# Seasandwpy/viso

Measured on AMD Instinct MI355X. Metric: stereo frames/sec at 1242x375 grey, 1/2/4/8 GPUs; pose RMSE vs reference, higher is better.
Workload: dtype f64

## Files before the change

viso_amd/csrc/context.hip:

```cpp
#include <algorithm>
#include <cstdio>
#include <cstring>
#include <new>
#include <vector>

#include "context.hpp"

using namespace viso;

namespace viso {

int DevBuf::ensure(size_t need) {
    if (need <= bytes) return VISO_OK;
    if (ptr) {
        VISO_HIP_CHECK(hipFree(ptr));
        ptr = nullptr;
        bytes = 0;
    }
    size_t b = std::max<size_t>(need, 256);
    VISO_HIP_CHECK(hipMalloc(&ptr, b));
    bytes = b;
    return VISO_OK;
}

// ... 60 lines not shown
int viso_create(const viso_params* p, int device, viso_ctx** out) {
    if (!p || !out) return VISO_ERR_ARG;
    *out = nullptr;
    if (p->width < 16 || p->height < 16 || p->width > kMaxWidth) return VISO_ERR_ARG;
    if (p->max_features <= 0 || p->max_features > 65536 || p->batch_frames <= 0) return VISO_ERR_ARG;
    if (p->precision != VISO_PRECISION_FAITHFUL && p->precision != VISO_PRECISION_FAST) return VISO_ERR_ARG;
    int rc = check_device_present();
    if (rc != VISO_OK) return rc;
    VISO_HIP_CHECK(hipSetDevice(device));
    viso_ctx* c = new (std::nothrow) viso_ctx();
    if (!c) return VISO_ERR_ARG;
    c->p = *p;
    c->device = device;
    if (const char* e = getenv("VISO_HOST_TIMES")) c->host_times.on = c->stage.timed = e[0] == '1';
    if (const char* e = getenv("VISO_HOST_TIMELINE")) c->dev_tl.on = e[0] == '1';
    c->geom = make_geom(p->width, p->height);
    if (c->create_streams() != VISO_OK) {
        delete c;
        return VISO_ERR_HIP;
    }
    rc = c->init();
    if (rc != VISO_OK) {
        viso_destroy(c);
        return rc;
    }
    *out = c;
    return VISO_OK;
}

int viso_destroy(viso_ctx* c) {
// ... 183 lines not shown
    if (rc) return rc;
    char* base = (char*)c->scratch_a.ptr;
    VISO_HIP_CHECK(hipMemcpyAsync(base + o_l, last_pyr, g.bytes, hipMemcpyHostToDevice, c->stream));
    VISO_HIP_CHECK(hipMemcpyAsync(base + o_c, cur_pyr, g.bytes, hipMemcpyHostToDevice, c->stream));
    if (n > 0)
        VISO_HIP_CHECK(hipMemcpyAsync(base + o_p, points, 24 * (size_t)n, hipMemcpyHostToDevice, c->stream));
    VISO_HIP_CHECK(hipMemcpyAsync(base + o_pl, pose_last, 96, hipMemcpyHostToDevice, c->stream));
    VISO_HIP_CHECK(hipMemcpyAsync(base + o_pio, pose_io, 96, hipMemcpyHostToDevice, c->stream));
    const double K[4] = {c->p.fx, c->p.fy, c->p.cx, c->p.cy};
    {
        TimedRegion t(c->timing, VISO_KERNEL_DIRECT, c->stream);
        launch_direct_pose(frame_from_base((const uint8_t*)(base + o_l), g),
                           frame_from_base((const uint8_t*)(base + o_c), g), g, K,
                           (const double*)(base + o_p), n, (const double*)(base + o_pl),
                           (const double*)(base + o_pio), direct_scratch_at(base + o_ds), nullptr,
                           (double*)(base + o_pio), nullptr, -1, c->stream, c->p.precision);
    }
    VISO_HIP_CHECK(hipGetLastError());
    VISO_HIP_CHECK(hipMemcpyAsync(pose_io, base + o_pio, 96, hipMemcpyDeviceToHost, c->stream));
    VISO_HIP_CHECK(hipStreamSynchronize(c->stream));
    return VISO_OK;
}

int viso_lk_align(viso_ctx* c, const uint8_t* kf_pyrs, const double* kf_poses, int32_t n_kf,
                  const uint8_t* cur_pyr, const double cur_pose[12], int32_t width, int32_t height,
                  const double* points, int32_t n, int32_t* pair_kf, uint8_t* success,
                  double* uv_before, double* uv_after) {
    if (!c || !kf_pyrs || !kf_poses || n_kf <= 0 || n_kf > kMaxKeyframes || !cur_pyr || !cur_pose ||
        n < 0)
        return VISO_ERR_ARG;
    if (int rc = c->settle()) return rc;
// ... 168 lines not shown
```

viso_amd/csrc/context.hpp:

```cpp
#pragma once

#include <chrono>
#include <deque>
#include <vector>

#include "../../include/viso/viso_c.h"
#include "geometry.hpp"
#include "kernels.hpp"
#include "staging.hpp"
#include "trace.hpp"

namespace viso {

struct DevBuf {
    void* ptr = nullptr;
    size_t bytes = 0;
    int ensure(size_t need);
    void release();
    template <class T>
    T* as() const { return (T*)ptr; }
};

struct Timing {
    bool enabled = false;
// ... 188 lines not shown
    viso::DevBuf map_pts;
    int n_map = 0;
    viso::DevBuf kf_poses;

    viso::DevBuf direct_buf;
    viso::DirectScratch direct{};
    viso::DevBuf direct_stats;
    std::vector<int> lk_pending;
    int lk_last_rows = 0;
    int lk_last_pts = 0;
    viso::DevBuf lk_pair, lk_succ, lk_before, lk_after;
    viso::DevBuf lk_tmpl, lk_tmpl_h, lk_tmpl_kf, lk_tmpl_uv;
    hipStream_t lk_stream = nullptr;
    hipEvent_t lk_ring[viso::kLkRing] = {};
    viso::HostStage stage;
    viso::HostTimes host_times;
    viso::DevTimeline dev_tl;
    hipStream_t up_stream = nullptr;
    int64_t epoch = 0;
    hipEvent_t epoch_evt[viso::kEpochRing] = {};
    int64_t epoch_rec_call[viso::kEpochRing] = {};
    int64_t epoch_nrec = 0;
    int64_t epoch_last_rec = -(1LL << 40);
    int wait_freed(int64_t fe, hipStream_t st);
    hipEvent_t epoch_now = nullptr;
    int end_epoch();
    int create_up_stream();
    int upload_host(int s, const uint8_t* grey, int32_t w, int32_t h, int32_t stride, bool pyramid);
    hipEvent_t geo_fork = nullptr, geo_join = nullptr;
    int64_t lk_seq = 0;
// ... 122 lines not shown
```

viso_amd/csrc/direct.hip:

```cpp
#include <algorithm>
#include <cstring>

#include "device_math.hpp"
#include "direct_solve.hpp"
#include "kernels.hpp"

#ifdef VISO_PROBE
constexpr int kPRing = 4096;
constexpr int kPSt = 16;
__device__ unsigned long long g_plog[kPRing][kPSt];
__device__ unsigned long long g_pexit[kPRing];
constexpr int kPRingB = 512;
__device__ unsigned long long g_pblk[kPRingB][256][4];
__device__ unsigned long long g_pwave[kPRingB][256][16];
#ifdef VISO_PROBE_PT
constexpr int kPtRing = 128, kPtBlocks = 32, kPtStamps = 5;
__device__ unsigned long long g_ppt[kPtRing][kPtBlocks][16][kPtStamps];
#define PPT(k)                                                                                       \
    do {                                                                                             \
        if (blockIdx.x < kPtBlocks && (threadIdx.x & 63) == 0)                                       \
            g_ppt[a.probe_seq & (kPtRing - 1)][blockIdx.x][threadIdx.x >> 6][(k)] =                  \
                __builtin_amdgcn_s_memrealtime();                                                    \
    } while (0)
#endif
// ... 266 lines not shown
            const int o = (iy - c.y0) * kCW + (ix - c.x0);
            const double d0 = (double)ld_lds_u8(win, o), d1 = (double)ld_lds_u8(win, o + 1);
            const double d2 = (double)ld_lds_u8(win, o + kCW), d3 = (double)ld_lds_u8(win, o + kCW + 1);
            const double xx = x - floor(x);
            const double yy = y - floor(y);
            return double((1 - xx) * (1 - yy) * d0 + xx * (1 - yy) * d1 + (1 - xx) * yy * d2 +
                          xx * yy * d3);
        }
    }
#ifdef VISO_PROBE
    PFB_ADD(w >= 1000 ? 0 : w >= 500 ? 1 : w >= 250 ? 2 : 3);
#endif
    return sample_px(img, w, h, x, y);
}

__device__ inline double point_quotients(const Intrinsics& K, const double* pose, const double* P, double scale,
                                         double* Q, double* qt) {
    const int lane = threadIdx.x & 63;
    double Pc[3];
    mat3_vec(pose, P, Pc);
    const double x = Pc[0] + pose[9], y = Pc[1] + pose[10], z = Pc[2] + pose[11];
    const double fx = K.fx * scale, fy = K.fy * scale;
    const double zz = z * z, xy = x * y;
    const double fxx = fx * x, fyy = fy * y;
    double c1, c2, den;
    if (qt) {
        if (lane == 0) {
            double2* t2 = reinterpret_cast<double2*>(qt);
            t2[0] = make_double2(x, y);
            t2[1] = make_double2(fx, -fx);
            t2[2] = make_double2(fxx, fy);
            t2[3] = make_double2(-fy, fyy);
            t2[4] = make_double2(1.0, xy);
            t2[5] = make_double2(z, zz);
        }
        __builtin_amdgcn_fence(__ATOMIC_RELEASE, "wavefront");
        __builtin_amdgcn_wave_barrier();
        __builtin_amdgcn_fence(__ATOMIC_ACQUIRE, "wavefront");
        constexpr unsigned long long kC1 = 0x557653433210ULL, kC2 = 0x091181090888ULL,
                                     kDen = 0xABBBAABBBAAAULL;
        const int l = lane < 12 ? lane : 11;
        c1 = qt[(kC1 >> (4 * l)) & 15];
        c2 = qt[(kC2 >> (4 * l)) & 15];
        den = qt[(kDen >> (4 * l)) & 15];
    } else {
        c1 = fy;
        c1 = lane == 0 ? x : c1;
        c1 = lane == 1 ? y : c1;
        c1 = lane == 2 ? fx : c1;
        c1 = (lane == 3 || lane == 4 || lane == 6) ? -fx : c1;
        c1 = lane == 5 ? fxx : c1;
        c1 = lane == 8 ? -fy : c1;
        c1 = lane == 9 ? fyy : c1;
        c2 = 1.0;
        c2 = (lane == 3 || lane == 5 || lane >= 11) ? x : c2;
        c2 = (lane == 4 || lane == 10) ? xy : c2;
        c2 = (lane == 6 || lane == 8 || lane == 9) ? y : c2;
        den = (lane <= 2 || lane == 6 || lane == 7 || lane >= 11) ? z : zz;
    }
    double q = (c1 * c2) / den;
    if (lane == 5) q = fx + q;
    if (lane == 9) q = -fy - q;
    Q[0] = readlane_f64(q, 0);
    Q[1] = readlane_f64(q, 1);
    return lane < 12 ? q : 0.0;
}

__device__ inline unsigned factored_sources() {
    const int k = threadIdx.x & 31;
    constexpr unsigned long long lo[4] = {0x43333ccccc222222ULL, 0x9888877777ccccccULL, 0x465436543c6543c2ULL,
                                          0x9ba98ba987ba987cULL};
    constexpr unsigned long long hi[4] = {0x26543c265544ULL, 0xcba987cbaa99ULL, 0xccccccc66565ULL,
                                          0x7777777bbabaULL};
    unsigned r = 0;
#pragma unroll
    for (int q = 0; q < 4; ++q)
        r |= (unsigned)((k < 16 ? lo[q] >> (4 * k) : hi[q] >> (4 * (k - 16))) & 15) << (8 * q);
// ... 11 lines not shown
        a[k] = ra + rb;
    }
    double ra, rb;
    permlane16_swap_f64(a[0], a[2], ra, rb);
    const double c0 = ra + rb;
    permlane16_swap_f64(a[1], a[1], ra, rb);
    const double c1 = ra + rb;
    double d = dsel(b3, c1, c0) + dpp_f64<0x128>(dsel(b3, c0, c1));
    const double r4 = dpp_f64<0x114>(d), l4 = dpp_f64<0x104>(d);
    d = d + dsel(b2, r4, l4);
    d = d + dpp_f64<0x4E>(d);
    d = d + dpp_f64<0xB1>(d);
    return d;
}

__device__ inline bool direct_point_rs(const DirectArgs& a, const LevelPair& fp, int lv,
                                       const double* cur_pose,
                                       const RefSample& r, const uint8_t* win, const CurWin& cw,
                                       double* out, int* idx, unsigned src_lanes, double* qt = nullptr) {
    const int lane = threadIdx.x & 63;
    const int px = (lane >> 3) - 4, py = (lane & 7) - 4;
    const double scale = kScale[lv];
    const int w = a.g.w[lv], h = a.g.h[lv];
    PPT(0);
    double Q[2];
    const double jq = point_quotients(a.K, cur_pose, r.P, scale, Q, qt);
    PPT(1);
    const double uc = scale * (Q[0] * a.K.fx + a.K.cx);
    const double vc = scale * (Q[1] * a.K.fy + a.K.cy);
    const double hp = 4.0;
    const bool good = r.ok && inside_px(uc - hp, vc - hp, w, h) && inside_px(uc + hp, vc + hp, w, h);
    if (!good) return false;
    const uint8_t* C = fp.cur;
    const double x = uc + px, y = vc + py;
    double error, g0, g1;
    const int fu = (int)floor(uc), fv = (int)floor(vc);
    if (__builtin_expect(cw.on && fu - 6 >= cw.x0 && fu + 5 <= cw.x0 + kCW - 2 && fv - 6 >= cw.y0 &&
                             fv + 5 <= cw.y0 + kCW - 2,
                         1)) {
        const bool one_binade = uc >= 6.0 && vc >= 6.0 &&
                                (__double_as_longlong(uc - 6.0) >> 52) == (__double_as_longlong(uc + 6.0) >> 52) &&
                                (__double_as_longlong(vc - 6.0) >> 52) == (__double_as_longlong(vc + 6.0) >> 52);
        if (__builtin_expect(one_binade, 1)) {
            const double xx = uc - floor(uc), yy = vc - floor(vc);
            const double w00 = (1 - xx) * (1 - yy), w10 = xx * (1 - yy), w01 = (1 - xx) * yy, w11 = xx * yy;
            const uint8_t* wb = win + ((fv + py - 1 - cw.y0) * kCW + (fu + px - 1 - cw.x0));
            auto tap = [&](int dx, int dy) { return (double)ld_lds_u8(wb, (dy + 1) * kCW + (dx + 1)); };
            const double tm0 = tap(-1, 0), t00 = tap(0, 0), t10 = tap(1, 0), t20 = tap(2, 0);
            const double tm1 = tap(-1, 1), t01 = tap(0, 1), t11 = tap(1, 1), t21 = tap(2, 1);
            const double t0m = tap(0, -1), t1m = tap(1, -1), t02 = tap(0, 2), t12 = tap(1, 2);
            auto bil = [&](double d0, double d1, double d2, double d3) {
                return double(w00 * d0 + w10 * d1 + w01 * d2 + w11 * d3);
            };
            error = r.lval - bil(t00, t10, t01, t11);
            g0 = 0.5 * (bil(t10, t20, t11, t21) - bil(tm0, t00, tm1, t01));
            g1 = 0.5 * (bil(t01, t11, t02, t12) - bil(t0m, t1m, t00, t10));
        } else {
            auto smp = [&](double sx, double sy) {
                const int o = ((int)sy - cw.y0) * kCW + ((int)sx - cw.x0);
                const double d0 = (double)ld_lds_u8(win, o), d1 = (double)ld_lds_u8(win, o + 1);
                const double d2 = (double)ld_lds_u8(win, o + kCW), d3 = (double)ld_lds_u8(win, o + kCW + 1);
                const double sxx = sx - floor(sx);
                const double syy = sy - floor(sy);
                return double((1 - sxx) * (1 - syy) * d0 + sxx * (1 - syy) * d1 + (1 - sxx) * syy * d2 +
                              sxx * syy * d3);
            };
            error = r.lval - smp(x, y);
            g0 = 0.5 * (smp(x + 1, y) - smp(x - 1, y));
            g1 = 0.5 * (smp(x, y + 1) - smp(x, y - 1));
        }
    } else {
        error = r.lval - sample_cw(C, w, h, x, y, win, cw);
        g0 = 0.5 * (sample_cw(C, w, h, x + 1, y, win, cw) - sample_cw(C, w, h, x - 1, y, win, cw));
        g1 = 0.5 * (sample_cw(C, w, h, x, y + 1, win, cw) - sample_cw(C, w, h, x, y - 1, win, cw));
    }
    PPT(2);
    const double leaf[6] = {g0 * g0, g0 * g1, g1 * g1, error * g0, error * g1, error * error};
    const double s = reduce_scatter_6_desc(leaf);
    PPT(3);
    const unsigned sa = src_lanes;
    const double p0a = bperm_f64(jq, (int)(sa & 0xff)), p1a = bperm_f64(jq, (int)((sa >> 8) & 0xff));
    const double p0b = bperm_f64(jq, (int)((sa >> 16) & 0xff)), p1b = bperm_f64(jq, (int)(sa >> 24));
    const double S0 = readlane_f64(s, 0), S1 = readlane_f64(s, 8), S2 = readlane_f64(s, 16);
    const double S3 = readlane_f64(s, 32), S4 = readlane_f64(s, 40), S5 = readlane_f64(s, 48);
    double o;
    if (lane < 21)
        o = (S0 * (p0a * p0b) + S1 * (p0a * p1b + p1a * p0b)) + S2 * (p1a * p1b);
    else if (lane < 27)
        o = S3 * p0a + S4 * p1a;
    else
        o = S5;
    *out = o;
    *idx = lane < kSums ? lane : -1;
    PPT(4);
    return true;
}

__device__ inline float tap_f32(const uint8_t* __restrict__ img, long long n, long long i) {
    return (float)ld_u8_or0(img, n, i);
}

__device__ inline bool direct_point_fast(const DirectArgs& a, const LevelPair& fp, int lv, const double* cur_pose,
                                         const double* P, float lval, const uint8_t* win, const CurWin& cw,
                                         float* out, int* idx) {
    const int lane = threadIdx.x & 63;
    const int px = (lane >> 3) - 4, py = (lane & 7) - 4;
    const double scale = kScale[lv];
    const int w = a.g.w[lv], h = a.g.h[lv];
    double Pc[3];
// ... 216 lines not shown
        const uint32_t t = pf.taps[j][lane];
        r.t0 = (int)(t & 0xff);
        r.t1 = (int)((t >> 8) & 0xff);
        r.t2 = (int)((t >> 16) & 0xff);
        r.t3 = (int)(t >> 24);
    } else {
        const uint8_t* img = fp.last;
        const long long n = (long long)w * (long long)h;
        r.t0 = ld_u8_or0(img, n, base);
        r.t1 = ld_u8_or0(img, n, base + 1);
        r.t2 = ld_u8_or0(img, n, base + w);
        r.t3 = ld_u8_or0(img, n, base + w + 1);
    }
}

constexpr unsigned kSrcHere = 0xffffffffu;

template <bool FAST, bool LV16 = false, int W = kWaves>
__device__ void direct_tile_pf(const DirectArgs& a, const LevelPair& fp, int lv, const double* cur_pose, int b,
                               const PfLds& pf, bool merged, double* part, int* good, double* s_pts,
                               int* s_good, int* s_cnt = nullptr, double* s_qt = nullptr,
                               unsigned src_in = kSrcHere) {
    const int wave = wave_id(), lane = threadIdx.x & 63;
    int first, T;
    tile_range(a, b, &first, &T);
    int good_cnt = 0;
    const unsigned src_lanes = FAST ? 0u : src_in != kSrcHere ? src_in : factored_sources();
    for (int local = wave; local < T; local += W) {
        const int i = first + local;
        double f = 0.0;
        int idx = -1;
        bool ok = false;
        if (i < a.n) {
            RefSample r;
            if (merged) {
                merged_ref(a, fp, lv, pf, local, r);
                if (!FAST) ref_finish(r);
            } else if (!FAST) {
                pf_ref(pf, local, r);
            } else {
                r.P[0] = pf.P[local][0];
                r.P[1] = pf.P[local][1];
// ... 8 lines not shown
                r.t3 = (int)(t >> 24);
            }
            CurWin cw;
            cw.x0 = pf.cw[local][0];
            cw.y0 = pf.cw[local][1];
            cw.on = pf.cw[local][2] != 0;
            if (FAST) {
                float ff = 0.0f;
                if (r.ok) {
                    const uint32_t t = (uint32_t)r.t0 | ((uint32_t)r.t1 << 8) | ((uint32_t)r.t2 << 16) |
                                       ((uint32_t)r.t3 << 24);
                    const float lval = (LV16 && !merged) ? (float)pf.lv16[local][lane] : fast_lval(t, r.ur, r.vr);
                    ok = direct_point_fast(a, fp, lv, cur_pose, r.P, lval, pf.win[local], cw, &ff, &idx);
                }
                f = (double)ff;
            } else {
                ok = direct_point_rs(a, fp, lv, cur_pose, r, pf.win[local], cw, &f, &idx, src_lanes,
                                     s_qt ? s_qt + 12 * wave : nullptr);
            }
        }
        if (!ok) {
            if (lane < kSums) s_pts[local * kSums + lane] = 0.0;
        } else if ((!FAST || lane < 32) && idx >= 0) {
            s_pts[local * kSums + idx] = f;
        }
        good_cnt += ok ? 1 : 0;
    }
    if (lane == 0 && good_cnt) atomicAdd(s_good, good_cnt);
#ifdef VISO_PROBE
    if (threadIdx.x == 0 && blockIdx.x < 256) g_pblk[a.probe_seq & (kPRingB - 1)][blockIdx.x][2] = __builtin_amdgcn_s_memrealtime();
// ... 137 lines not shown
            for (int k = 0; k < 7; ++k) a.s.state[kLevels * kStateStride + k] = L.state[k];
            if (a.prev_pose_out) store_frame_pose(a.prev_pose_out, s_last, a.prev_ready);
            log_pose(a.prev_log, a.prev_log_host, a.prev_log_index, s_last);
            log_frame(a.flog, a.prev_log_index, L);
        }
        double q[4];
        quat_from_matrix(s_last, q);
        for (int k = 0; k < 4; ++k) L.state[k] = q[k];
        L.state[4] = s_last[9];
        L.state[5] = s_last[10];
        L.state[6] = s_last[11];
    }
    state_to_pose(L.state, s_pose);
}

template <bool FAST>
__global__ __launch_bounds__(kThreads, 4) void direct_level_kernel(const double* __restrict__ pre_part,
                                                                 const int* __restrict__ pre_good, int pre_hdr,
                                                                 DirectArgs a) {
    PROBE_DECL();
    __builtin_amdgcn_s_setprio(1);
    __shared__ SolveLds L;
    __shared__ double s_pose[12];
    __shared__ double s_last[12];
    __shared__ double s_pts[kMaxTile * kSums];
    __shared__ int s_good;
    __shared__ int s_cnt;
    __shared__ int s_arrive;
    __shared__ PfLds s_pf;
#ifndef VISO_NO_QT
    __shared__ __attribute__((aligned(16))) double s_qt[FAST ? 2 : kWaves * 12];
    double* const qt = FAST ? nullptr : s_qt;
#else
    double* const qt = nullptr;
#endif
    const int lv = a.level;
    const bool merged = a.merged && lv == kLevels - 1;
    const int prev = lv + 1;
    const bool solve = prev < kLevels || merged;
    const int sl = merged ? 0 : prev;
    const int t = threadIdx.x, wave = t >> 6, lane = t & 63;
    const bool tiles = lv >= 0 && (int)blockIdx.x < a.n_tiles;
    double v[kSums];
    int gg = 0;
    if (((pre_hdr >> 16) & 1) && t < 256) load_partials(pre_part, pre_good, pre_hdr & 0xffff, v, gg);
    const bool pf_wave = !solve || (wave & 3) != 0;
    double st[7];
    if (t == 256 || (solve && tiles && pf_wave)) {
        if (!solve) {
            quat_from_matrix(a.pose_seed, st);
// ... 3 lines not shown
        } else {
#pragma unroll
            for (int k = 0; k < 7; ++k) st[k] = a.s.state[sl * kStateStride + k];
        }
    }
    if (t == 0) {
        s_arrive = 0;
        s_good = 0;
        s_cnt = 0;
#ifdef VISO_PROBE
        for (int k = 0; k < kPSt; ++k) pst[k] = 0;
        pst[0] = probe_t0;
        if (blockIdx.x < 256) g_pblk[a.probe_seq & (kPRingB - 1)][blockIdx.x][0] = probe_t0;
#endif
    }
    lds_barrier();

    if (t == 256) {
        for (int k = 0; k < 7; ++k) {
            L.state[k] = st[k];
            L.best[k] = st[k];
        }
        L.cost = 0.0;
        L.last_cost = 0.0;
        L.cont = 0;
        asm volatile("s_waitcnt lgkmcnt(0)" ::: "memory");
        atomicAdd(&s_arrive, 1);
    }
    if (solve && t < 256) {
        int idx;
// ... 82 lines not shown
        if (lv < 0 && a.pose_out) {
            store_frame_pose(a.pose_out, s_pose, a.ready);
            log_pose(a.log, a.log_host, a.log_index, s_pose);
            log_frame(a.flog, a.log_index, L);
        }
    }
    if (blockIdx.x == 0 && t == 0 && merged)
        for (int k = 0; k < 7; ++k) a.s.state[lv * kStateStride + k] = L.state[k];
    if (tiles) {
        LevelPair fp = level_pair(a.fp, lv);
        if (merged) fp.pose_last = s_last;
        double pose[12];
#pragma unroll
        for (int k = 0; k < 12; ++k) pose[k] = s_pose[k];
        direct_tile_pf<FAST>(a, fp, lv, pose, blockIdx.x, s_pf, merged, a.s.part + (size_t)lv * kMaxTiles * kSums,
                       a.s.good + lv * kMaxTiles, s_pts, &s_good, &s_cnt, qt, src_lanes);
    }
#ifdef VISO_PROBE
    __syncthreads();
    const unsigned long long t_exit = __builtin_amdgcn_s_memrealtime();
    const int slot = a.probe_seq & (kPRing - 1);
    if (t == 0 && blockIdx.x < 256) g_pblk[a.probe_seq & (kPRingB - 1)][blockIdx.x][3] = t_exit;
    if (blockIdx.x == 0 && t == 0) {
        pst[11] = t_exit;
        pst[15] = (unsigned long long)(lv + 1) | ((unsigned long long)merged << 8) |
                  ((unsigned long long)a.n_tiles << 16);
        for (int k = 0; k < kPSt; ++k) g_plog[slot][k] = pst[k];
    }
#endif
}

// ... 420 lines not shown
    }
    a.s = s;
    a.stats = stats;
    a.log_index = -1;
    a.prev_log_index = -1;
    return a;
}
}

bool direct_fits_background() { return kThreads <= 768; }

void launch_direct_levels(const FrameDev& last_pyr, const FrameDev& cur_pyr, const PyrGeom& g,
                          const double K[4], const double* points, int n,
                          const double* pose_last12, const double* pose_seed12,
                          const DirectScratch& s, double* stats, const DirectPrev* merge,
                          hipStream_t stream, int precision, bool bg) {
    DirectArgs a = direct_args(last_pyr, cur_pyr, g, K, points, n, pose_last12, pose_seed12, s,
                               stats, precision == VISO_PRECISION_FAST);
    if (merge) {
        a.merged = 1;
        a.prev.last = merge->last;
        a.prev.cur = merge->cur;
        a.prev.pose_last = merge->pose_last12;
        a.prev_pose_out = merge->pose_out;
        a.prev_log = merge->log;
        a.prev_log_index = merge->log ? merge->log_index : -1;
        a.prev_log_host = merge->log ? merge->log_host : nullptr;
        a.prev_ready = merge->ready;
        a.flog = merge->log ? merge->flog : nullptr;
    }
    const int grid = a.n_tiles > 0 ? a.n_tiles : 1;
    for (int level = kLevels - 1; level >= 0; --level) {
        a.level = level;
        a.probe_seq = next_probe_seq();
        const bool merged = a.merged && level == kLevels - 1;
        const bool solve = level + 1 < kLevels || merged;
        const int sl = merged ? 0 : level + 1;
        const double* pp = solve ? a.s.part + (size_t)sl * kMaxTiles * kSums : nullptr;
        const int* pg = solve ? a.s.good + sl * kMaxTiles : nullptr;
        const int hdr = a.n_tiles | (solve ? 1 << 16 : 0) | (bg ? kHdrBg : 0);
        if (precision == VISO_PRECISION_FAST)
            direct_level_kernel<true><<<grid, kThreads, 0, stream>>>(pp, pg, hdr, a);
        else
            direct_level_kernel<false><<<grid, kThreads, 0, stream>>>(pp, pg, hdr, a);
        a.merged = 0;
    }
}

void launch_direct_final(const FrameDev& last_pyr, const FrameDev& cur_pyr, const PyrGeom& g,
                         const double K[4], const double* points, int n,
                         const double* pose_last12, const DirectScratch& s, double* stats,
                         double* pose_out, double* log, int log_index, hipStream_t stream, int precision,
                         int* ready, double* log_host, double* flog) {
    DirectArgs a = direct_args(last_pyr, cur_pyr, g, K, points, n, pose_last12, pose_last12, s,
                               stats, precision == VISO_PRECISION_FAST);
    a.pose_out = pose_out;
    a.ready = ready;
// ... 103 lines not shown
            else
                rig_level_kernel<false, true><<<gl, kRigThreads, 0, stream>>>(psc, pad, hdr, t01, t23, ra);
        } else if (fast) {
            rig_level_kernel<true, false><<<gl, kRigThreads, 0, stream>>>(psc, pad, hdr, t01, t23, ra);
        } else {
            rig_level_kernel<false, false><<<gl, kRigThreads, 0, stream>>>(psc, pad, hdr, t01, t23, ra);
        }
    }
    return 0;
}

void launch_direct_pose(const FrameDev& last_pyr, const FrameDev& cur_pyr, const PyrGeom& g,
                        const double K[4], const double* points, int n,
                        const double* pose_last12, const double* pose_seed12,
                        const DirectScratch& s, double* stats, double* pose_out, double* log,
                        int log_index, hipStream_t stream, int precision) {
    launch_direct_levels(last_pyr, cur_pyr, g, K, points, n, pose_last12, pose_seed12, s, stats,
                         nullptr, stream, precision);
    launch_direct_final(last_pyr, cur_pyr, g, K, points, n, pose_last12, s, stats, pose_out, log,
                        log_index, stream, precision);
}

}

#ifdef VISO_PROBE
extern "C" int viso_debug_probe_ring(unsigned long long* log, unsigned long long* exits, int cap, int* n_launches,
                                     int reset) {
    using namespace viso;
    static unsigned long long hlog[kPRing][kPSt], hexit[kPRing];
    if (hipDeviceSynchronize() != hipSuccess) return -2;
    if (hipMemcpyFromSymbol(hlog, HIP_SYMBOL(g_plog), sizeof(hlog)) != hipSuccess) return -2;
    if (hipMemcpyFromSymbol(hexit, HIP_SYMBOL(g_pexit), sizeof(hexit)) != hipSuccess) return -2;
    const int n = (int)g_probe_host_seq;
// ... 86 lines not shown
```

viso_amd/csrc/frame.hip:

```cpp
#include <algorithm>
#include <cstdio>
#include <cstring>
#include <vector>

#include "context.hpp"

using namespace viso;

namespace {

void eigen_inverse3(const double* m, double* inv) {
    auto M = [&](int i, int j) { return m[3 * i + j]; };
    auto cof = [&](int i, int j) {
        int i1 = (i + 1) % 3, i2 = (i + 2) % 3, j1 = (j + 1) % 3, j2 = (j + 2) % 3;
        return M(i1, j1) * M(i2, j2) - M(i1, j2) * M(i2, j1);
    };
    double c0[3] = {cof(0, 0), cof(1, 0), cof(2, 0)};
    double det = (c0[0] * M(0, 0) + c0[1] * M(1, 0)) + c0[2] * M(2, 0);
    double invdet = 1.0 / det;
    inv[0] = c0[0] * invdet;
    inv[1] = c0[1] * invdet;
    inv[2] = c0[2] * invdet;
    inv[3] = cof(0, 1) * invdet;
    inv[4] = cof(1, 1) * invdet;
// ... 1082 lines not shown
                if (dpend) {
                    m.last = frame(dpend_last);
                    m.cur = frame(dpend_cur);
                    m.pose_last12 = pose_of(dpend_last);
                    m.pose_out = pose_of(dpend_cur);
                    m.log = dpend_log >= 0 ? (double*)pose_log.ptr : nullptr;
                    m.log_index = dpend_log;
                    m.ready = bg_ready(dpend_bg);
                    m.log_host = log_host(dpend_log);
                    m.flog = flog();
                }
                dev_tl.mark(frames, 3, stream);
                launch_direct_levels(frame(last_slot), frame(cur), g, K, (const double*)map_pts.ptr,
                                     n_map, pose_of(last_slot), pose_of(last_slot), direct,
                                     (double*)direct_stats.ptr, dpend ? &m : nullptr, stream, p.precision,
                                     bg_active);
                dev_tl.mark(frames, 4, stream);
            }
            if (dpend) {
                drop(dpend_cur);
                drop(dpend_last);
            }
            dpend = true;
            dpend_cur = cur;
            dpend_last = last_slot;
            hold(cur);
            hold(last_slot);
            dpend_log = log ? n_poses : -1;
            slots[(size_t)cur].log_index = dpend_log;
            dpend_bg = bg_active ? bg_cur : -1;
            if (log) ++n_poses;
// ... 454 lines not shown
```

viso_amd/csrc/kernels.hpp:

```cpp
#pragma once

#include "../../include/viso/viso_c.h"
#include "common.hpp"

namespace viso {

void launch_pyramid(const PyrGeom& g, uint8_t* base, int n_images, size_t img_stride,
                    hipStream_t stream);
constexpr int kPyrBatch = 128;
struct FastScratch {
    int* cnt = nullptr;
    int* tot = nullptr;
    int* lst = nullptr;
};

struct FastPre {
    const uint8_t* img = nullptr;
    int w = 0, h = 0, thresh = 0;
    FastScratch s;
    bool done = false;
};

struct PyrOwn {
    int img;
// ... 185 lines not shown

constexpr int kMaxMapPoints = 16384;
struct DirectScratch {
    double* part = nullptr;
    int* good = nullptr;
    double* state = nullptr;
    double* cont_part = nullptr;
    int* cont_good = nullptr;
};
size_t direct_scratch_bytes();
DirectScratch direct_scratch_at(void* base);
void launch_direct_pose(const FrameDev& last, const FrameDev& cur, const PyrGeom& g,
                        const double K[4], const double* points, int n,
                        const double* pose_last12, const double* pose_seed12,
                        const DirectScratch& s, double* stats, double* pose_out, double* log,
                        int log_index, hipStream_t stream, int precision = VISO_PRECISION_FAITHFUL);
struct DirectPrev {
    FrameDev last, cur;
    const double* pose_last12;
    double* pose_out;
    double* log;
    int log_index;
    int* ready = nullptr;
    double* log_host = nullptr;
    double* flog = nullptr;
};
bool direct_fits_background();
void launch_direct_levels(const FrameDev& last, const FrameDev& cur, const PyrGeom& g,
                          const double K[4], const double* points, int n,
                          const double* pose_last12, const double* pose_seed12,
                          const DirectScratch& s, double* stats, const DirectPrev* merge,
                          hipStream_t stream, int precision = VISO_PRECISION_FAITHFUL, bool bg = false);
void launch_direct_final(const FrameDev& last, const FrameDev& cur, const PyrGeom& g,
                         const double K[4], const double* points, int n,
                         const double* pose_last12, const DirectScratch& s, double* stats,
                         double* pose_out, double* log, int log_index, hipStream_t stream,
                         int precision = VISO_PRECISION_FAITHFUL, int* ready = nullptr,
                         double* log_host = nullptr, double* flog = nullptr);
constexpr int kMaxRigCams = 4;
struct RigCamDev {
    FrameDev last, cur;
    const double* points;
    int n;
    const double* pose_last12;
    double E[12];
    const double* Ad;
    void* scratch;
// ... 16 lines not shown
```

Measured before the change: 20750.

## Offload per-point projection and classification to helper waves in direct tile kernel

Adds a specialised direct_level_kernel variant in which two helper waves precompute each tile point's projection quotients, bilinear weights and window classification into LDS. The remaining waves spin on ready flags and consume these values instead of recomputing the projection per point. It is enabled by default when the tile size falls in a narrow range, and can be switched off with an environment variable. The aim is to take the serial projection math off the critical path of each point wave, at the cost of extra LDS, spin-waiting and fewer waves doing sampling work.

```diff
diff --git a/viso_amd/csrc/context.hip b/viso_amd/csrc/context.hip
--- a/viso_amd/csrc/context.hip
+++ b/viso_amd/csrc/context.hip
@@ -98,6 +98,7 @@
     c->device = device;
     if (const char* e = getenv("VISO_HOST_TIMES")) c->host_times.on = c->stage.timed = e[0] == '1';
     if (const char* e = getenv("VISO_HOST_TIMELINE")) c->dev_tl.on = e[0] == '1';
+    if (const char* e = getenv("VISO_DIRECT_SCALAR_PASS")) c->direct_scalar_pass = e[0] != '0';
     c->geom = make_geom(p->width, p->height);
     if (c->create_streams() != VISO_OK) {
         delete c;
@@ -311,7 +312,8 @@
                            frame_from_base((const uint8_t*)(base + o_c), g), g, K,
                            (const double*)(base + o_p), n, (const double*)(base + o_pl),
                            (const double*)(base + o_pio), direct_scratch_at(base + o_ds), nullptr,
-                           (double*)(base + o_pio), nullptr, -1, c->stream, c->p.precision);
+                           (double*)(base + o_pio), nullptr, -1, c->stream, c->p.precision,
+                           c->direct_scalar_pass);
     }
     VISO_HIP_CHECK(hipGetLastError());
     VISO_HIP_CHECK(hipMemcpyAsync(pose_io, base + o_pio, 96, hipMemcpyDeviceToHost, c->stream));
diff --git a/viso_amd/csrc/context.hpp b/viso_amd/csrc/context.hpp
--- a/viso_amd/csrc/context.hpp
+++ b/viso_amd/csrc/context.hpp
@@ -226,6 +226,7 @@
     hipStream_t lk_stream = nullptr;
     hipEvent_t lk_ring[viso::kLkRing] = {};
     viso::HostStage stage;
+    bool direct_scalar_pass = true;
     viso::HostTimes host_times;
     viso::DevTimeline dev_tl;
     hipStream_t up_stream = nullptr;
diff --git a/viso_amd/csrc/direct.hip b/viso_amd/csrc/direct.hip
--- a/viso_amd/csrc/direct.hip
+++ b/viso_amd/csrc/direct.hip
@@ -304,9 +304,38 @@
     return sample_px(img, w, h, x, y);
 }
 
-__device__ inline double point_quotients(const Intrinsics& K, const double* pose, const double* P, double scale,
-                                         double* Q, double* qt) {
-    const int lane = threadIdx.x & 63;
+__device__ inline double quotient_slot(const Intrinsics& K, const double* pose, const double* P, double scale, int k,
+                                       bool lead, double* qt) {
+    double Pc[3];
+    mat3_vec(pose, P, Pc);
+    const double x = Pc[0] + pose[9], y = Pc[1] + pose[10], z = Pc[2] + pose[11];
+    const double fx = K.fx * scale, fy = K.fy * scale;
+    const double zz = z * z, xy = x * y;
+    const double fxx = fx * x, fyy = fy * y;
+    if (lead) {
+        double2* t2 = reinterpret_cast<double2*>(qt);
+        t2[0] = make_double2(x, y);
+        t2[1] = make_double2(fx, -fx);
+        t2[2] = make_double2(fxx, fy);
+        t2[3] = make_double2(-fy, fyy);
+        t2[4] = make_double2(1.0, xy);
+        t2[5] = make_double2(z, zz);
+    }
+    __builtin_amdgcn_fence(__ATOMIC_RELEASE, "wavefront");
+    __builtin_amdgcn_wave_barrier();
+    __builtin_amdgcn_fence(__ATOMIC_ACQUIRE, "wavefront");
+    constexpr unsigned long long kC1 = 0x557653433210ULL, kC2 = 0x091181090888ULL, kDen = 0xABBBAABBBAAAULL;
+    const double c1 = qt[(kC1 >> (4 * k)) & 15];
+    const double c2 = qt[(kC2 >> (4 * k)) & 15];
+    const double den = qt[(kDen >> (4 * k)) & 15];
+    double q = (c1 * c2) / den;
+    if (k == 5) q = fx + q;
+    if (k == 9) q = -fy - q;
+    return q;
+}
+
+__device__ inline double quotient_select(const Intrinsics& K, const double* pose, const double* P, double scale,
+                                         int k) {
     double Pc[3];
     mat3_vec(pose, P, Pc);
     const double x = Pc[0] + pose[9], y = Pc[1] + pose[10], z = Pc[2] + pose[11];
@@ -314,43 +343,30 @@
     const double zz = z * z, xy = x * y;
     const double fxx = fx * x, fyy = fy * y;
     double c1, c2, den;
-    if (qt) {
-        if (lane == 0) {
-            double2* t2 = reinterpret_cast<double2*>(qt);
-            t2[0] = make_double2(x, y);
-            t2[1] = make_double2(fx, -fx);
-            t2[2] = make_double2(fxx, fy);
-            t2[3] = make_double2(-fy, fyy);
-            t2[4] = make_double2(1.0, xy);
-            t2[5] = make_double2(z, zz);
-        }
-        __builtin_amdgcn_fence(__ATOMIC_RELEASE, "wavefront");
-        __builtin_amdgcn_wave_barrier();
-        __builtin_amdgcn_fence(__ATOMIC_ACQUIRE, "wavefront");
-        constexpr unsigned long long kC1 = 0x557653433210ULL, kC2 = 0x091181090888ULL,
-                                     kDen = 0xABBBAABBBAAAULL;
-        const int l = lane < 12 ? lane : 11;
-        c1 = qt[(kC1 >> (4 * l)) & 15];
-        c2 = qt[(kC2 >> (4 * l)) & 15];
-        den = qt[(kDen >> (4 * l)) & 15];
-    } else {
-        c1 = fy;
-        c1 = lane == 0 ? x : c1;
-        c1 = lane == 1 ? y : c1;
-        c1 = lane == 2 ? fx : c1;
-        c1 = (lane == 3 || lane == 4 || lane == 6) ? -fx : c1;
-        c1 = lane == 5 ? fxx : c1;
-        c1 = lane == 8 ? -fy : c1;
-        c1 = lane == 9 ? fyy : c1;
-        c2 = 1.0;
-        c2 = (lane == 3 || lane == 5 || lane >= 11) ? x : c2;
-        c2 = (lane == 4 || lane == 10) ? xy : c2;
-        c2 = (lane == 6 || lane == 8 || lane == 9) ? y : c2;
-        den = (lane <= 2 || lane == 6 || lane == 7 || lane >= 11) ? z : zz;
-    }
+    c1 = fy;
+    c1 = k == 0 ? x : c1;
+    c1 = k == 1 ? y : c1;
+    c1 = k == 2 ? fx : c1;
+    c1 = (k == 3 || k == 4 || k == 6) ? -fx : c1;
+    c1 = k == 5 ? fxx : c1;
+    c1 = k == 8 ? -fy : c1;
+    c1 = k == 9 ? fyy : c1;
+    c2 = 1.0;
+    c2 = (k == 3 || k == 5 || k == 11) ? x : c2;
+    c2 = (k == 4 || k == 10) ? xy : c2;
+    c2 = (k == 6 || k == 8 || k == 9) ? y : c2;
+    den = (k <= 2 || k == 6 || k == 7 || k == 11) ? z : zz;
     double q = (c1 * c2) / den;
-    if (lane == 5) q = fx + q;
-    if (lane == 9) q = -fy - q;
+    if (k == 5) q = fx + q;
+    if (k == 9) q = -fy - q;
+    return q;
+}
+
+__device__ inline double point_quotients(const Intrinsics& K, const double* pose, const double* P, double scale,
+                                         double* Q, double* qt) {
+    const int lane = threadIdx.x & 63;
+    const int k = lane < 12 ? lane : 11;
+    const double q = qt ? quotient_slot(K, pose, P, scale, k, lane == 0, qt) : quotient_select(K, pose, P, scale, k);
     Q[0] = readlane_f64(q, 0);
     Q[1] = readlane_f64(q, 1);
     return lane < 12 ? q : 0.0;
@@ -392,66 +408,68 @@
     return d;
 }
 
-__device__ inline bool direct_point_rs(const DirectArgs& a, const LevelPair& fp, int lv,
-                                       const double* cur_pose,
-                                       const RefSample& r, const uint8_t* win, const CurWin& cw,
-                                       double* out, int* idx, unsigned src_lanes, double* qt = nullptr) {
+enum : int {
+    kClsOut = 0,
+    kClsShared = 1,
+    kClsStraddle = 2,
+    kClsSample = 3,
+};
+
+__device__ inline bool patch_in_window(bool on, int x0, int y0, int fu, int fv) {
+    return on && fu - 6 >= x0 && fu + 5 <= x0 + kCW - 2 && fv - 6 >= y0 && fv + 5 <= y0 + kCW - 2;
+}
+
+__device__ inline bool patch_one_binade(double uc, double vc) {
+    return uc >= 6.0 && vc >= 6.0 &&
+           (__double_as_longlong(uc - 6.0) >> 52) == (__double_as_longlong(uc + 6.0) >> 52) &&
+           (__double_as_longlong(vc - 6.0) >> 52) == (__double_as_longlong(vc + 6.0) >> 52);
+}
+
+__device__ inline void samples_shared(const uint8_t* win, const CurWin& cw, int fu, int fv, double w00, double w10,
+                                      double w01, double w11, double lval, double& error, double& g0,
+                                      double& g1) {
     const int lane = threadIdx.x & 63;
     const int px = (lane >> 3) - 4, py = (lane & 7) - 4;
-    const double scale = kScale[lv];
-    const int w = a.g.w[lv], h = a.g.h[lv];
-    PPT(0);
-    double Q[2];
-    const double jq = point_quotients(a.K, cur_pose, r.P, scale, Q, qt);
-    PPT(1);
-    const double uc = scale * (Q[0] * a.K.fx + a.K.cx);
-    const double vc = scale * (Q[1] * a.K.fy + a.K.cy);
-    const double hp = 4.0;
-    const bool good = r.ok && inside_px(uc - hp, vc - hp, w, h) && inside_px(uc + hp, vc + hp, w, h);
-    if (!good) return false;
-    const uint8_t* C = fp.cur;
-    const double x = uc + px, y = vc + py;
-    double error, g0, g1;
-    const int fu = (int)floor(uc), fv = (int)floor(vc);
-    if (__builtin_expect(cw.on && fu - 6 >= cw.x0 && fu + 5 <= cw.x0 + kCW - 2 && fv - 6 >= cw.y0 &&
-                             fv + 5 <= cw.y0 + kCW - 2,
-                         1)) {
-        const bool one_binade = uc >= 6.0 && vc >= 6.0 &&
-                                (__double_as_longlong(uc - 6.0) >> 52) == (__double_as_longlong(uc + 6.0) >> 52) &&
-                                (__double_as_longlong(vc - 6.0) >> 52) == (__double_as_longlong(vc + 6.0) >> 52);
-        if (__builtin_expect(one_binade, 1)) {
-            const double xx = uc - floor(uc), yy = vc - floor(vc);
-            const double w00 = (1 - xx) * (1 - yy), w10 = xx * (1 - yy), w01 = (1 - xx) * yy, w11 = xx * yy;
-            const uint8_t* wb = win + ((fv + py - 1 - cw.y0) * kCW + (fu + px - 1 - cw.x0));
-            auto tap = [&](int dx, int dy) { return (double)ld_lds_u8(wb, (dy + 1) * kCW + (dx + 1)); };
-            const double tm0 = tap(-1, 0), t00 = tap(0, 0), t10 = tap(1, 0), t20 = tap(2, 0);
-            const double tm1 = tap(-1, 1), t01 = tap(0, 1), t11 = tap(1, 1), t21 = tap(2, 1);
-            const double t0m = tap(0, -1), t1m = tap(1, -1), t02 = tap(0, 2), t12 = tap(1, 2);
-            auto bil = [&](double d0, double d1, double d2, double d3) {
-                return double(w00 * d0 + w10 * d1 + w01 * d2 + w11 * d3);
-            };
-            error = r.lval - bil(t00, t10, t01, t11);
-            g0 = 0.5 * (bil(t10, t20, t11, t21) - bil(tm0, t00, tm1, t01));
-            g1 = 0.5 * (bil(t01, t11, t02, t12) - bil(t0m, t1m, t00, t10));
-        } else {
-            auto smp = [&](double sx, double sy) {
-                const int o = ((int)sy - cw.y0) * kCW + ((int)sx - cw.x0);
-                const double d0 = (double)ld_lds_u8(win, o), d1 = (double)ld_lds_u8(win, o + 1);
-                const double d2 = (double)ld_lds_u8(win, o + kCW), d3 = (double)ld_lds_u8(win, o + kCW + 1);
-                const double sxx = sx - floor(sx);
-                const double syy = sy - floor(sy);
-                return double((1 - sxx) * (1 - syy) * d0 + sxx * (1 - syy) * d1 + (1 - sxx) * syy * d2 +
-                              sxx * syy * d3);
-            };
-            error = r.lval - smp(x, y);
-            g0 = 0.5 * (smp(x + 1, y) - smp(x - 1, y));
-            g1 = 0.5 * (smp(x, y + 1) - smp(x, y - 1));
-        }
-    } else {
-        error = r.lval - sample_cw(C, w, h, x, y, win, cw);
-        g0 = 0.5 * (sample_cw(C, w, h, x + 1, y, win, cw) - sample_cw(C, w, h, x - 1, y, win, cw));
-        g1 = 0.5 * (sample_cw(C, w, h, x, y + 1, win, cw) - sample_cw(C, w, h, x, y - 1, win, cw));
-    }
+    const uint8_t* wb = win + ((fv + py - 1 - cw.y0) * kCW + (fu + px - 1 - cw.x0));
+    auto tap = [&](int dx, int dy) { return (double)ld_lds_u8(wb, (dy + 1) * kCW + (dx + 1)); };
+    const double tm0 = tap(-1, 0), t00 = tap(0, 0), t10 = tap(1, 0), t20 = tap(2, 0);
+    const double tm1 = tap(-1, 1), t01 = tap(0, 1), t11 = tap(1, 1), t21 = tap(2, 1);
+    const double t0m = tap(0, -1), t1m = tap(1, -1), t02 = tap(0, 2), t12 = tap(1, 2);
+    auto bil = [&](double d0, double d1, double d2, double d3) {
+        return double(w00 * d0 + w10 * d1 + w01 * d2 + w11 * d3);
+    };
+    error = lval - bil(t00, t10, t01, t11);
+    g0 = 0.5 * (bil(t10, t20, t11, t21) - bil(tm0, t00, tm1, t01));
+    g1 = 0.5 * (bil(t01, t11, t02, t12) - bil(t0m, t1m, t00, t10));
+}
+
+__device__ inline void samples_straddle(const uint8_t* win, const CurWin& cw, double x, double y, double lval,
+                                        double& error, double& g0, double& g1) {
+    auto smp = [&](double sx, double sy) {
+        const int o = ((int)sy - cw.y0) * kCW + ((int)sx - cw.x0);
+        const double d0 = (double)ld_lds_u8(win, o), d1 = (double)ld_lds_u8(win, o + 1);
+        const double d2 = (double)ld_lds_u8(win, o + kCW), d3 = (double)ld_lds_u8(win, o + kCW + 1);
+        const double sxx = sx - floor(sx);
+        const double syy = sy - floor(sy);
+        return double((1 - sxx) * (1 - syy) * d0 + sxx * (1 - syy) * d1 + (1 - sxx) * syy * d2 +
+                      sxx * syy * d3);
+    };
+    error = lval - smp(x, y);
+    g0 = 0.5 * (smp(x + 1, y) - smp(x - 1, y));
+    g1 = 0.5 * (smp(x, y + 1) - smp(x, y - 1));
+}
+
+__device__ inline void samples_each(const uint8_t* __restrict__ C, int w, int h, const uint8_t* win,
+                                    const CurWin& cw, double x, double y, double lval, double& error, double& g0,
+                                    double& g1) {
+    error = lval - sample_cw(C, w, h, x, y, win, cw);
+    g0 = 0.5 * (sample_cw(C, w, h, x + 1, y, win, cw) - sample_cw(C, w, h, x - 1, y, win, cw));
+    g1 = 0.5 * (sample_cw(C, w, h, x, y + 1, win, cw) - sample_cw(C, w, h, x, y - 1, win, cw));
+}
+
+__device__ inline void point_sums_factored(double error, double g0, double g1, double jq, unsigned src_lanes,
+                                           double* out, int* idx) {
+    const int lane = threadIdx.x & 63;
     PPT(2);
     const double leaf[6] = {g0 * g0, g0 * g1, g1 * g1, error * g0, error * g1, error * error};
     const double s = reduce_scatter_6_desc(leaf);
@@ -471,6 +489,85 @@
     *out = o;
     *idx = lane < kSums ? lane : -1;
     PPT(4);
+}
+
+constexpr int kSpHelpers = 2;
+constexpr int kSpPerHelper = 5;
+constexpr int kSpLanes = 12;
+constexpr int kSpPoints = kSpHelpers * kSpPerHelper;
+static_assert(kSpPoints == kWaves - kSpHelpers, "the helpers are the two waves above the tile's points");
+static_assert(kSpPerHelper * kSpLanes <= 64, "a helper's points fit its lanes");
+
+struct SpLds {
+    double v[kSpPoints][16];
+    int cls[kSpPoints][4];
+    int ready[kSpPoints];
+};
+
+__device__ inline bool direct_point_rs(const DirectArgs& a, const LevelPair& fp, int lv,
+                                       const double* cur_pose,
+                                       const RefSample& r, const uint8_t* win, const CurWin& cw,
+                                       double* out, int* idx, unsigned src_lanes, double* qt = nullptr) {
+    const int lane = threadIdx.x & 63;
+    const int px = (lane >> 3) - 4, py = (lane & 7) - 4;
+    const double scale = kScale[lv];
+    const int w = a.g.w[lv], h = a.g.h[lv];
+    PPT(0);
+    double Q[2];
+    const double jq = point_quotients(a.K, cur_pose, r.P, scale, Q, qt);
+    PPT(1);
+    const double uc = scale * (Q[0] * a.K.fx + a.K.cx);
+    const double vc = scale * (Q[1] * a.K.fy + a.K.cy);
+    const double hp = 4.0;
+    const bool good = r.ok && inside_px(uc - hp, vc - hp, w, h) && inside_px(uc + hp, vc + hp, w, h);
+    if (!good) return false;
+    const double x = uc + px, y = vc + py;
+    double error, g0, g1;
+    const int fu = (int)floor(uc), fv = (int)floor(vc);
+    if (__builtin_expect(patch_in_window(cw.on, cw.x0, cw.y0, fu, fv), 1)) {
+        if (__builtin_expect(patch_one_binade(uc, vc), 1)) {
+            const double xx = uc - floor(uc), yy = vc - floor(vc);
+            const double w00 = (1 - xx) * (1 - yy), w10 = xx * (1 - yy), w01 = (1 - xx) * yy, w11 = xx * yy;
+            samples_shared(win, cw, fu, fv, w00, w10, w01, w11, r.lval, error, g0, g1);
+        } else {
+            samples_straddle(win, cw, x, y, r.lval, error, g0, g1);
+        }
+    } else {
+        samples_each(fp.cur, w, h, win, cw, x, y, r.lval, error, g0, g1);
+    }
+    point_sums_factored(error, g0, g1, jq, src_lanes, out, idx);
+    return true;
+}
+
+__device__ inline bool direct_point_sp(const DirectArgs& a, const LevelPair& fp, int lv, const RefSample& r,
+                                       const uint8_t* win, const CurWin& cw, const SpLds& sp, int j, double* out,
+                                       int* idx, unsigned src_lanes) {
+    const int lane = threadIdx.x & 63;
+    const int px = (lane >> 3) - 4, py = (lane & 7) - 4;
+    PPT(0);
+    while (__hip_atomic_load(&sp.ready[j], __ATOMIC_RELAXED, __HIP_MEMORY_SCOPE_WORKGROUP) == 0)
+        __builtin_amdgcn_s_sleep(1);
+    __builtin_amdgcn_fence(__ATOMIC_ACQUIRE, "workgroup");
+    const double ql = sp.v[j][lane < 12 ? lane : 11];
+    const double jq = lane < 12 ? ql : 0.0;
+    const double2 s01 = reinterpret_cast<const double2*>(&sp.v[j][12])[0];
+    const double2 s23 = reinterpret_cast<const double2*>(&sp.v[j][12])[1];
+    const int4 ci = *reinterpret_cast<const int4*>(sp.cls[j]);
+    const int cls = __builtin_amdgcn_readfirstlane(ci.x);
+    const int fu = __builtin_amdgcn_readfirstlane(ci.y), fv = __builtin_amdgcn_readfirstlane(ci.z);
+    PPT(1);
+    if (!(r.ok && cls != kClsOut)) return false;
+    double error, g0, g1;
+    if (__builtin_expect(cls == kClsShared, 1)) {
+        samples_shared(win, cw, fu, fv, s01.x, s01.y, s23.x, s23.y, r.lval, error, g0, g1);
+    } else {
+        const double x = s01.x + px, y = s01.y + py;
+        if (cls == kClsStraddle)
+            samples_straddle(win, cw, x, y, r.lval, error, g0, g1);
+        else
+            samples_each(fp.cur, a.g.w[lv], a.g.h[lv], win, cw, x, y, r.lval, error, g0, g1);
+    }
+    point_sums_factored(error, g0, g1, jq, src_lanes, out, idx);
     return true;
 }
 
@@ -717,18 +814,60 @@
     }
 }
 
+__device__ inline void scalar_pass(const DirectArgs& a, int lv, const double* cur_pose, const PfLds& pf, int first,
+                                   int T, int helper, SpLds& sp) {
+    const int lane = threadIdx.x & 63;
+    const bool act = lane < kSpPerHelper * kSpLanes;
+    const int p = act ? lane / kSpLanes : kSpPerHelper - 1;
+    const int k = act ? lane - kSpLanes * p : kSpLanes - 1;
+    const int j = kSpPerHelper * helper + p;
+    const bool valid = act && j < T && first + j < a.n;
+    const double scale = kScale[lv];
+    const int w = a.g.w[lv], h = a.g.h[lv];
+    const double P[3] = {pf.P[j][0], pf.P[j][1], pf.P[j][2]};
+    const double q = quotient_select(a.K, cur_pose, P, scale, k);
+    const double Q0 = bperm_f64(q, kSpLanes * p), Q1 = bperm_f64(q, kSpLanes * p + 1);
+    const double uc = scale * (Q0 * a.K.fx + a.K.cx);
+    const double vc = scale * (Q1 * a.K.fy + a.K.cy);
+    const double hp = 4.0;
+    const bool in = inside_px(uc - hp, vc - hp, w, h) && inside_px(uc + hp, vc + hp, w, h);
+    const int fu = (int)floor(uc), fv = (int)floor(vc);
+    const bool whole = patch_in_window(pf.cw[j][2] != 0, pf.cw[j][0], pf.cw[j][1], fu, fv);
+    const int cls = !in ? kClsOut : !whole ? kClsSample : patch_one_binade(uc, vc) ? kClsShared : kClsStraddle;
+    const double xx = uc - floor(uc), yy = vc - floor(vc);
+    const double w00 = (1 - xx) * (1 - yy), w10 = xx * (1 - yy), w01 = (1 - xx) * yy, w11 = xx * yy;
+    const bool shared = cls == kClsShared;
+    if (valid) {
+        sp.v[j][k] = q;
+        if (k == 0) {
+            double2* v2 = reinterpret_cast<double2*>(&sp.v[j][12]);
+            v2[0] = make_double2(shared ? w00 : uc, shared ? w10 : vc);
+            v2[1] = make_double2(w01, w11);
+            *reinterpret_cast<int4*>(sp.cls[j]) = make_int4(cls, fu, fv, 0);
+        }
+    }
+    __builtin_amdgcn_fence(__ATOMIC_RELEASE, "workgroup");
+    if (valid && k == 0) __hip_atomic_store(&sp.ready[j], 1, __ATOMIC_RELAXED, __HIP_MEMORY_SCOPE_WORKGROUP);
+}
+
 constexpr unsigned kSrcHere = 0xffffffffu;
 
 template <bool FAST, bool LV16 = false, int W = kWaves>
 __device__ void direct_tile_pf(const DirectArgs& a, const LevelPair& fp, int lv, const double* cur_pose, int b,
                                const PfLds& pf, bool merged, double* part, int* good, double* s_pts,
                                int* s_good, int* s_cnt = nullptr, double* s_qt = nullptr,
-                               unsigned src_in = kSrcHere) {
+                               unsigned src_in = kSrcHere, SpLds* sp = nullptr) {
     const int wave = wave_id(), lane = threadIdx.x & 63;
     int first, T;
     tile_range(a, b, &first, &T);
     int good_cnt = 0;
     const unsigned src_lanes = FAST ? 0u : src_in != kSrcHere ? src_in : factored_sources();
+    const bool sp_on = !FAST && W == kWaves && sp && s_cnt && T > kSpPoints - kSpHelpers && T <= kSpPoints;
+    if (sp_on && wave >= kSpPoints) {
+        __builtin_amdgcn_s_setprio(3);
+        scalar_pass(a, lv, cur_pose, pf, first, T, wave - kSpPoints, *sp);
+        __builtin_amdgcn_s_setprio(1);
+    }
     for (int local = wave; local < T; local += W) {
         const int i = first + local;
         double f = 0.0;
@@ -767,6 +906,8 @@
                     ok = direct_point_fast(a, fp, lv, cur_pose, r.P, lval, pf.win[local], cw, &ff, &idx);
                 }
                 f = (double)ff;
+            } else if (sp_on) {
+                ok = direct_point_sp(a, fp, lv, r, pf.win[local], cw, *sp, local, &f, &idx, src_lanes);
             } else {
                 ok = direct_point_rs(a, fp, lv, cur_pose, r, pf.win[local], cw, &f, &idx, src_lanes,
                                      s_qt ? s_qt + 12 * wave : nullptr);
@@ -934,7 +1075,7 @@
     state_to_pose(L.state, s_pose);
 }
 
-template <bool FAST>
+template <bool FAST, bool SP = false>
 __global__ __launch_bounds__(kThreads, 4) void direct_level_kernel(const double* __restrict__ pre_part,
                                                                  const int* __restrict__ pre_good, int pre_hdr,
                                                                  DirectArgs a) {
@@ -954,6 +1095,7 @@
 #else
     double* const qt = nullptr;
 #endif
+    __shared__ __attribute__((aligned(16))) SpLds s_sp;
     const int lv = a.level;
     const bool merged = a.merged && lv == kLevels - 1;
     const int prev = lv + 1;
@@ -987,6 +1129,7 @@
         if (blockIdx.x < 256) g_pblk[a.probe_seq & (kPRingB - 1)][blockIdx.x][0] = probe_t0;
 #endif
     }
+    if (SP && t >= kThreads - kSpPoints) s_sp.ready[kThreads - 1 - t] = 0;
     lds_barrier();
 
     if (t == 256) {
@@ -1099,7 +1242,8 @@
 #pragma unroll
         for (int k = 0; k < 12; ++k) pose[k] = s_pose[k];
         direct_tile_pf<FAST>(a, fp, lv, pose, blockIdx.x, s_pf, merged, a.s.part + (size_t)lv * kMaxTiles * kSums,
-                       a.s.good + lv * kMaxTiles, s_pts, &s_good, &s_cnt, qt, src_lanes);
+                       a.s.good + lv * kMaxTiles, s_pts, &s_good, &s_cnt, qt, src_lanes,
+                       SP ? &s_sp : nullptr);
     }
 #ifdef VISO_PROBE
     __syncthreads();
@@ -1550,7 +1694,7 @@
                           const double K[4], const double* points, int n,
                           const double* pose_last12, const double* pose_seed12,
                           const DirectScratch& s, double* stats, const DirectPrev* merge,
-                          hipStream_t stream, int precision, bool bg) {
+                          hipStream_t stream, int precision, bool bg, bool scalar_pass) {
     DirectArgs a = direct_args(last_pyr, cur_pyr, g, K, points, n, pose_last12, pose_seed12, s,
                                stats, precision == VISO_PRECISION_FAST);
     if (merge) {
@@ -1577,6 +1721,8 @@
         const int hdr = a.n_tiles | (solve ? 1 << 16 : 0) | (bg ? kHdrBg : 0);
         if (precision == VISO_PRECISION_FAST)
             direct_level_kernel<true><<<grid, kThreads, 0, stream>>>(pp, pg, hdr, a);
+        else if (scalar_pass && a.tile > kSpPoints - kSpHelpers && a.tile <= kSpPoints)
+            direct_level_kernel<false, true><<<grid, kThreads, 0, stream>>>(pp, pg, hdr, a);
         else
             direct_level_kernel<false><<<grid, kThreads, 0, stream>>>(pp, pg, hdr, a);
         a.merged = 0;
@@ -1710,9 +1856,9 @@
                         const double K[4], const double* points, int n,
                         const double* pose_last12, const double* pose_seed12,
                         const DirectScratch& s, double* stats, double* pose_out, double* log,
-                        int log_index, hipStream_t stream, int precision) {
+                        int log_index, hipStream_t stream, int precision, bool scalar_pass) {
     launch_direct_levels(last_pyr, cur_pyr, g, K, points, n, pose_last12, pose_seed12, s, stats,
-                         nullptr, stream, precision);
+                         nullptr, stream, precision, false, scalar_pass);
     launch_direct_final(last_pyr, cur_pyr, g, K, points, n, pose_last12, s, stats, pose_out, log,
                         log_index, stream, precision);
 }
diff --git a/viso_amd/csrc/frame.hip b/viso_amd/csrc/frame.hip
--- a/viso_amd/csrc/frame.hip
+++ b/viso_amd/csrc/frame.hip
@@ -1120,7 +1120,7 @@
                 launch_direct_levels(frame(last_slot), frame(cur), g, K, (const double*)map_pts.ptr,
                                      n_map, pose_of(last_slot), pose_of(last_slot), direct,
                                      (double*)direct_stats.ptr, dpend ? &m : nullptr, stream, p.precision,
-                                     bg_active);
+                                     bg_active, direct_scalar_pass);
                 dev_tl.mark(frames, 4, stream);
             }
             if (dpend) {
diff --git a/viso_amd/csrc/kernels.hpp b/viso_amd/csrc/kernels.hpp
--- a/viso_amd/csrc/kernels.hpp
+++ b/viso_amd/csrc/kernels.hpp
@@ -223,7 +223,8 @@
                         const double K[4], const double* points, int n,
                         const double* pose_last12, const double* pose_seed12,
                         const DirectScratch& s, double* stats, double* pose_out, double* log,
-                        int log_index, hipStream_t stream, int precision = VISO_PRECISION_FAITHFUL);
+                        int log_index, hipStream_t stream, int precision = VISO_PRECISION_FAITHFUL,
+                        bool scalar_pass = true);
 struct DirectPrev {
     FrameDev last, cur;
     const double* pose_last12;
@@ -239,7 +240,8 @@
                           const double K[4], const double* points, int n,
                           const double* pose_last12, const double* pose_seed12,
                           const DirectScratch& s, double* stats, const DirectPrev* merge,
-                          hipStream_t stream, int precision = VISO_PRECISION_FAITHFUL, bool bg = false);
+                          hipStream_t stream, int precision = VISO_PRECISION_FAITHFUL, bool bg = false,
+                          bool scalar_pass = true);
 void launch_direct_final(const FrameDev& last, const FrameDev& cur, const PyrGeom& g,
                          const double K[4], const double* points, int n,
                          const double* pose_last12, const DirectScratch& s, double* stats,
```

After: 21160, median of 6. 1.02x the previous value.
